# emdgroup/tnmf

Hardware: NVIDIA B200
Metric: sample-iterations/sec for 2-D shift-NMF MU at 1/2/4/8 B200; % of roofline (higher is better)
Workload: dtype f32

## Files before the change

### tnmf_b200/csrc/tc_gradw_ts.cu

```cuda
#include "tc_common.cuh"

namespace tnmf {
namespace tc {
namespace gwt {

using tiled::ceil_div;
using tiled::Geo2;
using tiled::round_up;

constexpr int kCT = 64;
constexpr int kNB = 16;
constexpr int kWorkers = 256;
#ifndef TNMF_GW_ISSUERS
#define TNMF_GW_ISSUERS 2
#endif
constexpr int kIssuers = TNMF_GW_ISSUERS;
constexpr int kThreads = 32 * (8 + kIssuers + 4);
constexpr int kEpoch = 8;
constexpr int kMaxAStages = 4;
constexpr int kRingMax = 24;
constexpr int kRawMax = 4;
constexpr int kMaxSmem = 226 * 1024;

struct Plan {
    int KPL;
    int TXP, RW, RWp, rawX, raw_floats, nraw;
    int KS, n_sub, n_astages, a_col0, NA;
    int RS, NRr, ring_floats;
    int tiles;
    long long total, quota, units;
    int round_robin;
    int grid;
    size_t smem;
};

struct Args {
    const float *V, *R, *H;
    float *partials;
    int m0;
};

bool make_plan(const Geo2 &g, Plan &p) {
    p = Plan();
    if (g.AY < 1 || g.AY > 14) return false;
    p.KPL = g.C * g.AX;
    if (p.KPL > 64) return false;
    p.NA = kNB * g.AY;
    const int spare = 512 - 2 * p.NA;
#ifdef TNMF_GW_KS16
    if (spare >= 2 * 32) p.KS = 16;
#else
    if (spare >= 2 * 64) p.KS = 32;
#endif
    else if (spare >= 2 * 32) p.KS = 16;
    else return false;
    p.n_sub = kCT / p.KS;
    p.n_astages = spare / (2 * p.KS);
    if (p.n_astages > kMaxAStages) p.n_astages = kMaxAStages;
    p.n_astages &= ~1;
    p.a_col0 = 2 * p.NA;
    p.TXP = g.TX + g.AX - 1;
    p.RW = kCT + g.AX - 1;
    p.RWp = p.RW + 1;
    while ((p.RWp - g.AX) % 32 != 0) ++p.RWp;
    p.rawX = round_up(g.C * p.RWp, 32);
    p.raw_floats = 2 * p.rawX + 128;
    p.nraw = ceil_div(2 * g.C * p.RW, kWorkers);
    if (p.nraw > kRawMax) return false;
    const size_t fixed = (size_t)2 * p.raw_floats * 4 + 1024;
    for (p.RS = kRingMax; p.RS >= g.AY + 1; --p.RS) {
        p.NRr = (p.RS + g.AY - 1) * kNB;
        p.ring_floats = (p.NRr * 4 + 4) * (kCT / 4);
        if (fixed + (size_t)2 * p.ring_floats * 4 <= (size_t)kMaxSmem) break;
    }
    if (p.RS < g.AY + 1) return false;
    p.smem = fixed + (size_t)2 * p.ring_floats * 4;
    const long long cols = (long long)g.N * p.TXP;
    if (cols <= 0 || cols >= (1ll << 31) - kCT) return false;
    p.tiles = (int)((cols + kCT - 1) / kCT);
    const int sms = tma::sm_count();
    p.total = (long long)p.tiles * g.TY;
    p.quota = (p.total + sms - 1) / sms;
    const long long min_quota = g.TY < 8 ? g.TY : 8;
    if (p.quota < min_quota) p.quota = min_quota;
    const long long whole = (p.tiles + sms - 1) / sms * (long long)g.TY;
    p.round_robin = (double)whole <= 1.1 * (double)(p.quota + 2 * (g.AY - 1));
    if (p.round_robin) {
        p.quota = g.TY;
        p.grid = p.tiles < sms ? p.tiles : sms;
        p.units = p.tiles;
        return true;
    }
    p.grid = (int)((p.total + p.quota - 1) / p.quota);
    p.units = (long long)p.grid * ((p.quota + g.TY - 2) / g.TY + 1);
    return true;
}

struct Unit {
    int tile, ty0, ty1, r_lo, r_hi;
};
__device__ __forceinline__ Unit make_unit(long long u, const Geo2 &g, const Plan &p) {
    Unit w;
    const long long b = u % p.grid, k = u / p.grid;
    const long long lo = p.round_robin ? u * (long long)g.TY : b * p.quota, hi = min(lo + p.quota, p.total);
    w.tile = p.round_robin ? (int)u : (int)(lo / g.TY + k);
    const long long t0 = (long long)w.tile * g.TY;
    const long long s0 = max(lo, t0), s1 = min(hi, t0 + g.TY);
    w.ty0 = s1 > s0 ? (int)(s0 - t0) : 0;
    w.ty1 = s1 > s0 ? (int)(s1 - t0) : 0;
    w.r_lo = max(0, w.ty0 - g.offy);
    w.r_hi = min(g.DY - 1, w.ty1 - 1 - g.offy + g.AY - 1);
    return w;
}

template <int KS>
__global__ void __launch_bounds__(kThreads, 1) gradw_ts_kernel(const Geo2 g, const Plan p, const Args a) {
    extern __shared__ __align__(128) float smem[];
    __shared__ __align__(8) unsigned long long a_full[kMaxAStages], a_empty[kMaxAStages], h_full[kRingMax], h_free[kRingMax],
        set_done[2], set_free[2];
    __shared__ unsigned tmem_base_s;
    constexpr int CPT = KS / 2;
    const int tid = threadIdx.x, warp = __shfl_sync(0xffffffffu, tid >> 5, 0), lane = tid & 31;
    const int AY = g.AY, AX = g.AX, C = g.C, RS = p.RS, RW = p.RW;
    float *ring_hi = smem, *ring_lo = smem + p.ring_floats;
    float *raw = ring_lo + p.ring_floats;

    if (tid == 0) {
        for (int s = 0; s < p.n_astages; ++s) { mbar_init(&a_full[s], 8); mbar_init(&a_empty[s], kIssuers); }
        for (int s = 0; s < kRingMax; ++s) { mbar_init(&h_full[s], kWorkers); mbar_init(&h_free[s], kIssuers); }
        for (int s = 0; s < 2; ++s) { mbar_init(&set_done[s], kIssuers); mbar_init(&set_free[s], 128); }
        mbar_fence_init();
    }
    if (warp == 8) tmem_alloc(&tmem_base_s, 512);
    for (int idx = tid; idx < 2 * p.raw_floats; idx += kThreads) raw[idx] = 0.f;
    tc_fence_before();
    __syncthreads();
    tc_fence_after();
    const unsigned tmem_base = tmem_base_s;
    if (warp < 4) {
        for (int c = 0; c < 512; c += 16) tmem_st16_zero(tmem_base + ((unsigned)(warp * 32) << 16) + (unsigned)c);
        tmem_st_wait();
    }
    tc_fence_before();
    __syncthreads();
    tc_fence_after();

    const long long count = (long long)g.M * C * AY * AX;

    if (warp < 8) {
        const int quarter = warp & 3, half = warp >> 2;
        const int L = quarter * 32 + lane;
        const int X = L >> 6, k = L & 63;
        const bool live = k < p.KPL;
        const bool warp_live = ((quarter * 32) & 63) < p.KPL;
        const int src_off = live ? X * p.rawX + (k / AX) * p.RWp + (k % AX) : 2 * p.rawX + 16;
        const unsigned t_lane = tmem_base + ((unsigned)(quarter * 32) << 16) + (unsigned)(p.a_col0 + half * CPT);
        int st = 0;
        unsigned ph = 0, buf = 0;
        TC_PROF_DECL(empty); TC_PROF_DECL(hfree); TC_PROF_DECL(bar); TC_PROF_DECL(total);
#ifdef TNMF_TC_PROFILE
        prof_total = -clock64();
#endif
        const long long plane = (long long)g.DY * g.DX;
        const int raw_count = 2 * C * RW;
        const int h_ml = tid >> 4, h_cg = tid & 15;
        int slot_new = 0;
        unsigned wraps = 0;
        for (long long u = blockIdx.x; u < p.units; u += gridDim.x) {
            const Unit w = make_unit(u, g, p);
            if (w.ty0 >= w.ty1) break;
            long long roff[kRawMax];
            int rdst[kRawMax];
#pragma unroll
            for (int e = 0; e < kRawMax; ++e) {
                roff[e] = -1;
                rdst[e] = -1;
                const int q = tid + kWorkers * e;
                if (e < p.nraw && q < raw_count) {
                    const int Xq = q / (C * RW), qq = q - Xq * (C * RW);
                    const int c = qq / RW, xr = qq - c * RW;
                    rdst[e] = Xq * p.rawX + c * p.RWp + xr;
                    const long long J = (long long)w.tile * kCT + xr;
                    const int n = (int)(J / p.TXP);
                    const int x = (int)(J - (long long)n * p.TXP) - g.offx;
                    if (n < g.N && (unsigned)x < (unsigned)g.DX) roff[e] = ((long long)n * C + c) * plane + x;
                }
            }
            long long hoff[4];
#pragma unroll
            for (int e = 0; e < 4; ++e) {
                const long long J = (long long)w.tile * kCT + 4 * h_cg + e;
                const int n = (int)(J / p.TXP);
                const int xv = (int)(J - (long long)n * p.TXP);
                hoff[e] = (n < g.N && xv < g.TX && a.m0 + h_ml < g.M)
                              ? (long long)n * g.hsn + (long long)(a.m0 + h_ml) * g.hsm + xv : -1;
            }
            float rv[kRawMax];
            auto load_raw = [&](int r) {
#pragma unroll
                for (int e = 0; e < kRawMax; ++e) {
                    const float *src = ((tid + kWorkers * e) >= C * RW) ? a.R : a.V;
                    rv[e] = roff[e] >= 0 ? __ldg(src + (long long)r * g.DX + roff[e]) : 0.f;
                }
            };
            auto load_h = [&](int ty) {
                float4 hv;
                hv.x = hoff[0] >= 0 ? a.H[hoff[0] + (long long)ty * g.hsy] : 0.f;
                hv.y = hoff[1] >= 0 ? a.H[hoff[1] + (long long)ty * g.hsy] : 0.f;
                hv.z = hoff[2] >= 0 ? a.H[hoff[2] + (long long)ty * g.hsy] : 0.f;
                hv.w = hoff[3] >= 0 ? a.H[hoff[3] + (long long)ty * g.hsy] : 0.f;
                return hv;
            };
            float4 hv_next = make_float4(0.f, 0.f, 0.f, 0.f);
            int hv_row = -1;
            int next_new = w.ty0;
            load_raw(w.r_lo);
            for (int r = w.r_lo; r <= w.r_hi; ++r) {
                const int t_b = min(w.ty1 - 1, r + g.offy);
                unsigned new_slots = 0;
                for (; next_new <= t_b; ++next_new) {
                    const int slot = slot_new;
                    const float4 hv = next_new == hv_row ? hv_next : load_h(next_new);
                    if (wraps) TC_PROF_WAIT(hfree, mbar_wait_backoff(&h_free[slot], (wraps - 1u) & 1u, 40));
                    if (++slot_new == RS) { slot_new = 0; ++wraps; }
                    float4 hi, lo;
                    split_tf32(hv.x, hi.x, lo.x); split_tf32(hv.y, hi.y, lo.y);
                    split_tf32(hv.z, hi.z, lo.z); split_tf32(hv.w, hi.w, lo.w);
                    const int nrow = slot * kNB + h_ml;
                    const size_t o = (size_t)(nrow >> 3) * 32 + (size_t)h_cg * (p.NRr * 4 + 4) + (size_t)(nrow & 7) * 4;
                    *reinterpret_cast<float4 *>(ring_hi + o) = hi;
                    *reinterpret_cast<float4 *>(ring_lo + o) = lo;
                    if (slot < AY - 1) {
                        const size_t om = o + (size_t)RS * (kNB / 8) * 32;
                        *reinterpret_cast<float4 *>(ring_hi + om) = hi;
                        *reinterpret_cast<float4 *>(ring_lo + om) = lo;
                    }
                    new_slots |= 1u << slot;
                }
                if (new_slots) {
                    fence_proxy_async();
                    for (; new_slots; new_slots &= new_slots - 1) mbar_arrive(&h_full[__ffs(new_slots) - 1]);
                }
                float *rb = raw + (size_t)buf * p.raw_floats;
#pragma unroll
                for (int e = 0; e < kRawMax; ++e)
                    if (rdst[e] >= 0) rb[rdst[e]] = rv[e];
                if (r < w.r_hi) load_raw(r + 1);
                if (next_new < w.ty1) { hv_next = load_h(next_new); hv_row = next_new; }
                TC_PROF_WAIT(bar, asm volatile("bar.sync 1, 256;\n" ::: "memory"));
                const float *src = rb + src_off + half * CPT;
                for (int h = 0; h < kCT / KS; ++h) {
                    TC_PROF_WAIT(empty, mbar_wait_backoff(&a_empty[st], ph ^ 1u, 20));
                    tc_fence_after();
                    if (warp_live) {
                        float hi[CPT], lo[CPT];
#pragma unroll
                        for (int j = 0; j < CPT; ++j) split_tf32(src[h * KS + j], hi[j], lo[j]);
                        const unsigned t = t_lane + (unsigned)(st * 2 * KS);
                        if constexpr (CPT == 16) {
                            tmem_st16(t, hi);
                            tmem_st16(t + KS, lo);
                        } else {
                            tmem_st8(t, hi);
                            tmem_st8(t + KS, lo);
                        }
                        tmem_st_wait();
                    }
                    tc_fence_before();
                    __syncwarp();
                    if (lane == 0) mbar_arrive(&a_full[st]);
                    if (++st == p.n_astages) { st = 0; ph ^= 1u; }
                }
                buf ^= 1u;
            }
        }
#ifdef TNMF_TC_PROFILE
        prof_total += clock64();
        if (blockIdx.x == 0 && tid == 0)
            printf("gradw_ts workers: total %lld  wait a_empty %lld  wait h_free %lld  raw barrier %lld\n", prof_total, prof_empty,
                   prof_hfree, prof_bar);
#endif
    } else if (warp >= 8 + kIssuers) {
        int rows_done = 0;
        bool first_drain = true;
        TC_PROF_DECL(done); TC_PROF_DECL(total);
#ifdef TNMF_TC_PROFILE
        prof_total = -clock64();
#endif
        auto drain = [&](int e) {
            const int set = (int)(e & 1);
            const int l = (warp & 3) * 32 + lane;
            const int X = l >> 6, k = l & 63;
            const bool live = k < p.KPL;
            const int c = live ? k / AX : 0, ax = live ? k - c * AX : 0;
            float *slice = a.partials + (long long)blockIdx.x * 2 * count + (long long)X * count;
            const unsigned tbase = tmem_base + ((unsigned)((warp & 3) * 32) << 16) + (unsigned)(set * p.NA);
            float old_next[kNB];
#pragma unroll
            for (int ml = 0; ml < kNB; ++ml) old_next[ml] = 0.f;
            if (live && !first_drain) {
                const float *nx = slice + (((long long)a.m0 * C + c) * AY + (AY - 1)) * AX + ax;
#pragma unroll
                for (int ml = 0; ml < kNB; ++ml) old_next[ml] = a.m0 + ml < g.M ? __ldcg(nx + ml * (long long)C * AY * AX) : 0.f;
            }
            TC_PROF_WAIT(done, mbar_wait_backoff(&set_done[set], (unsigned)((e >> 1) & 1), 100));
            tc_fence_after();
            const long long mstride = (long long)C * AY * AX;
            float *dst_base = slice + (((long long)a.m0 * C + c) * AY) * AX + ax;
            for (int j = 0; j < AY; ++j) {
                float v[16], old[kNB];
#pragma unroll
                for (int ml = 0; ml < kNB; ++ml) old[ml] = old_next[ml];
                if (j + 1 < AY && live && !first_drain) {
                    const float *nx = dst_base + (long long)(AY - 2 - j) * AX;
#pragma unroll
                    for (int ml = 0; ml < kNB; ++ml) old_next[ml] = a.m0 + ml < g.M ? __ldcg(nx + ml * mstride) : 0.f;
                }
                tmem_ld16(tbase + (unsigned)(j * kNB), v);
                tmem_ld_wait();
                tmem_st16_zero(tbase + (unsigned)(j * kNB));
                if (live) {
                    float *dst0 = dst_base + (long long)(AY - 1 - j) * AX;
#pragma unroll
                    for (int ml = 0; ml < kNB; ++ml)
                        if (a.m0 + ml < g.M) __stcg(dst0 + ml * mstride, v[ml] + old[ml]);
                }
            }
            tmem_st_wait();
            tc_fence_before();
            mbar_arrive(&set_free[set]);
            first_drain = false;
        };
        for (long long u = blockIdx.x; u < p.units; u += gridDim.x) {
            const Unit w = make_unit(u, g, p);
            if (w.ty0 >= w.ty1) break;
            rows_done += w.r_hi - w.r_lo + 1;
        }
        const int n_epochs = (rows_done + kEpoch - 1) / kEpoch;
        for (int e = 0; e < n_epochs; ++e) drain(e);
#ifdef TNMF_TC_PROFILE
        prof_total += clock64();
        if (blockIdx.x == 0 && tid == 32 * (8 + kIssuers))
            printf("gradw_ts drainers: total %lld  wait set_done %lld  (%d epochs)\n", prof_total, prof_done, n_epochs);
#endif
    } else {
        const unsigned tmem_u = __shfl_sync(0xffffffffu, tmem_base, 0);
        const unsigned lbo_b = (unsigned)p.NRr * 16 + 16;
        const unsigned desc_hi = (128u >> 4) | (1u << 14);
        const unsigned b_lo_word = ((lbo_b >> 4) << 16);
        const unsigned ring_hi16 = __shfl_sync(0xffffffffu, smem_u32(ring_hi) >> 4, 0);
        const unsigned ring_lo16 = __shfl_sync(0xffffffffu, smem_u32(ring_lo) >> 4, 0);
        const unsigned b_step16 = (2 * lbo_b) >> 4;
        const int X = warp - 8;
        const int j_lo = (AY * X + kIssuers - 1) / kIssuers, j_hi = (AY * (X + 1) + kIssuers - 1) / kIssuers - 1;
        int st = 0;
        unsigned ph = 0;
        int rows_done = 0;
        int slot_new = 0, slot_out = 0, slot_a = 0;
        unsigned par_new = 0;
        TC_PROF_DECL(full); TC_PROF_DECL(hfull); TC_PROF_DECL(setfree); TC_PROF_DECL(total); TC_PROF_DECL(issue); TC_PROF_DECL(commit); TC_PROF_DECL(commit2);
#ifdef TNMF_TC_PROFILE
        prof_total = -clock64();
#endif
        for (long long u = blockIdx.x; u < p.units; u += gridDim.x) {
            const Unit w = make_unit(u, g, p);
            if (w.ty0 >= w.ty1) break;
            int next_new = w.ty0, next_out = w.ty0, win0 = w.ty0;
            slot_a = slot_new;
            for (int r = w.r_lo; r <= w.r_hi; ++r) {
                const int epoch = rows_done / kEpoch;
                if (rows_done % kEpoch == 0 && epoch >= 2) {
                    TC_PROF_WAIT(setfree, mbar_wait(&set_free[epoch & 1], (unsigned)(((epoch >> 1) - 1) & 1)));
                    tc_fence_after();
                }
                const unsigned tset = tmem_u + (unsigned)((epoch & 1) * p.NA);
                const int ay_hi = min(AY - 1, r + g.offy - w.ty0);
                const int t_a = r + g.offy - ay_hi, t_b = min(w.ty1 - 1, r + g.offy);
                const int j0 = r + g.offy - AY + 1;
                for (; next_new <= t_b; ++next_new) {
                    TC_PROF_WAIT(hfull, mbar_wait(&h_full[slot_new], par_new));
                    if (++slot_new == RS) { slot_new = 0; par_new ^= 1u; }
                }
                for (; win0 < t_a; ++win0)
                    if (++slot_a == RS) slot_a = 0;
                const int ta_x = max(t_a, j0 + j_lo), tb_x = min(t_b, j0 + j_hi);
                const int cnt = tb_x - ta_x + 1;
                const unsigned col0 = tset + (unsigned)((ta_x - j0) * kNB);
                const unsigned idesc0 = idesc_tf32(128, kNB * max(cnt, 1));
                const unsigned b0 = (unsigned)(slot_a + (ta_x - t_a)) * 16u;
                for (int h = 0; h < kCT / KS; ++h) {
                    TC_PROF_WAIT(full, mbar_wait(&a_full[st], ph));
                    tc_fence_after();
#ifdef TNMF_TC_PROFILE
                    const long long t_i = clock64();
#endif
                    const unsigned ta_hi = tmem_u + (unsigned)(p.a_col0 + st * 2 * KS), ta_lo = ta_hi + KS;
                    if (cnt > 0 && elect_one()) {
#pragma unroll
                        for (int ks = 0; ks < KS / 8; ++ks) {
                            const unsigned kb = (unsigned)(h * (KS / 8) + ks) * b_step16 + b0;
                            const unsigned long long b_hi = ((unsigned long long)desc_hi << 32) | (b_lo_word | (ring_hi16 + kb));
                            const unsigned long long b_lo = ((unsigned long long)desc_hi << 32) | (b_lo_word | (ring_lo16 + kb));
                            mma_tf32_ts(col0, ta_hi + 8u * ks, b_hi, idesc0, 1u);
                            mma_tf32_ts(col0, ta_lo + 8u * ks, b_hi, idesc0, 1u);
                            mma_tf32_ts(col0, ta_hi + 8u * ks, b_lo, idesc0, 1u);
                        }
                    }
                    __syncwarp();
#ifdef TNMF_TC_PROFILE
                    prof_issue += clock64() - t_i;
#endif
                    TC_PROF_WAIT(commit, mma_commit_elect(&a_empty[st]));
                    if (++st == p.n_astages) { st = 0; ph ^= 1u; }
                }
                for (; next_out < w.ty1 && min(g.DY - 1, next_out - g.offy + AY - 1) <= r; ++next_out) {
                    TC_PROF_WAIT(commit2, mma_commit_elect(&h_free[slot_out]));
                    if (++slot_out == RS) slot_out = 0;
                }
                if (++rows_done % kEpoch == 0) mma_commit_elect(&set_done[epoch & 1]);
            }
        }
        if (rows_done % kEpoch != 0) mma_commit_elect(&set_done[(rows_done / kEpoch) & 1]);
#ifdef TNMF_TC_PROFILE
        prof_total += clock64();
        if (blockIdx.x == 0 && lane == 0)
            printf("gradw_ts mma %d: total %lld  wait a_full %lld  wait h_full %lld  wait set_free %lld  issuing %lld  commit a_empty %lld  commit h_free %lld (%d rows)\n",
                   X, prof_total, prof_full, prof_hfull, prof_setfree, prof_issue, prof_commit, prof_commit2, rows_done);
#endif
        __syncwarp();
    }
    tc_fence_before();
    __syncthreads();
    if (warp == 8) tmem_dealloc(tmem_base, 512);
}

template <int KS>
static int launch(const Geo2 &g, const Plan &p, const Args &a, cudaStream_t st) {
    auto kern = gradw_ts_kernel<KS>;
    cudaError_t e = cudaFuncSetAttribute(kern, cudaFuncAttributeMaxDynamicSharedMemorySize, kMaxSmem);
    if (e != cudaSuccess) return status_from_cuda(e);
    kern<<<(unsigned)p.grid, kThreads, p.smem, st>>>(g, p, a);
    TNMF_CHECK_LAUNCH();
    return TNMF_OK;
}

}
}

bool tc_gradw_ts_supported(const Geo &g, int dtype) {
    if (!tc::rank2_ok(g, dtype)) return false;
    tc::gwt::Plan p;
    return tc::gwt::make_plan(tiled::make_geo2(g), p);
}

size_t tc_gradw_ts_workspace_bytes(const Geo &g) {
    tc::gwt::Plan p;
    if (!tc::gwt::make_plan(tiled::make_geo2(g), p)) return 0;
    return (size_t)p.grid * 2 * (size_t)g.M * g.C * g.A[1] * g.A[2] * sizeof(float);
}

int tc_gradient_w_ts(const Geo &g, const float *V, const float *R, const float *H, float *neg, float *pos, void *workspace,
                     size_t workspace_bytes, cudaStream_t st) {
    const tiled::Geo2 q = tiled::make_geo2(g);
    tc::gwt::Plan p;
    if (!tc::gwt::make_plan(q, p)) return TNMF_EUNSUPPORTED;
    const long long count = (long long)g.M * g.C * g.A[1] * g.A[2];
    if (!workspace || workspace_bytes < tc_gradw_ts_workspace_bytes(g)) return TNMF_EWORKSPACE;
    tc::gwt::Args a;
    a.V = V; a.R = R; a.H = H; a.partials = (float *)workspace;
    for (int m0 = 0; m0 < g.M; m0 += tc::gwt::kNB) {
        a.m0 = m0;
        const int s = p.KS == 32 ? tc::gwt::launch<32>(q, p, a, st) : tc::gwt::launch<16>(q, p, a, st);
        if (s) return s;
    }
    return finish_gradient_w<float>((const float *)workspace, p.grid, count, neg, pos, st);
}

int tc_gradw_ts_launches(const Geo &g) { return tiled::ceil_div(g.M, tc::gwt::kNB) + 1; }

}
```

Before: 34740.

## Pack hi/lo TF32 splits into separate TMEM lanes when KPL fits 32

```diff
diff --git a/tnmf_b200/csrc/tc_gradw_ts.cu b/tnmf_b200/csrc/tc_gradw_ts.cu
--- a/tnmf_b200/csrc/tc_gradw_ts.cu
+++ b/tnmf_b200/csrc/tc_gradw_ts.cu
@@ -21,9 +21,14 @@
 constexpr int kRingMax = 24;
 constexpr int kRawMax = 4;
 constexpr int kMaxSmem = 226 * 1024;
+constexpr int kMaxLeft = 1;
+constexpr int kLeftRing = 16;
+constexpr int kXchg = 2 * 2 * kNB * 32;
+constexpr int kDrainers = 128;
 
 struct Plan {
     int KPL;
+    int hl, side;
     int TXP, RW, RWp, rawX, raw_floats, nraw;
     int KS, n_sub, n_astages, a_col0, NA;
     int RS, NRr, ring_floats;
@@ -40,24 +45,28 @@
     int m0;
 };
 
-bool make_plan(const Geo2 &g, Plan &p) {
+bool make_plan(const Geo2 &g, Plan &p, bool hl_ok = true) {
     p = Plan();
     if (g.AY < 1 || g.AY > 14) return false;
     p.KPL = g.C * g.AX;
     if (p.KPL > 64) return false;
+    p.hl = hl_ok && p.KPL <= 32 + kMaxLeft;
+    p.side = p.hl && p.KPL > 32;
     p.NA = kNB * g.AY;
     const int spare = 512 - 2 * p.NA;
+    if (p.hl) p.KS = 32;
 #ifdef TNMF_GW_KS16
-    if (spare >= 2 * 32) p.KS = 16;
+    else if (spare >= 2 * 32) p.KS = 16;
 #else
-    if (spare >= 2 * 64) p.KS = 32;
+    else if (spare >= 2 * 64) p.KS = 32;
 #endif
     else if (spare >= 2 * 32) p.KS = 16;
     else return false;
     p.n_sub = kCT / p.KS;
-    p.n_astages = spare / (2 * p.KS);
+    p.n_astages = spare / ((p.hl ? 1 : 2) * p.KS);
     if (p.n_astages > kMaxAStages) p.n_astages = kMaxAStages;
     p.n_astages &= ~1;
+    if (p.n_astages < 2) return false;
     p.a_col0 = 2 * p.NA;
     p.TXP = g.TX + g.AX - 1;
     p.RW = kCT + g.AX - 1;
@@ -67,13 +76,13 @@
     p.raw_floats = 2 * p.rawX + 128;
     p.nraw = ceil_div(2 * g.C * p.RW, kWorkers);
     if (p.nraw > kRawMax) return false;
-    const size_t fixed = (size_t)2 * p.raw_floats * 4 + 1024;
+    const size_t fixed = (size_t)2 * p.raw_floats * 4 + 1024 + (p.hl ? kXchg * 4 : 0) + (p.side ? kLeftRing * 128 * 4 : 0);
     for (p.RS = kRingMax; p.RS >= g.AY + 1; --p.RS) {
         p.NRr = (p.RS + g.AY - 1) * kNB;
         p.ring_floats = (p.NRr * 4 + 4) * (kCT / 4);
         if (fixed + (size_t)2 * p.ring_floats * 4 <= (size_t)kMaxSmem) break;
     }
-    if (p.RS < g.AY + 1) return false;
+    if (p.RS < g.AY + 1) return p.hl && make_plan(g, p, false);
     p.smem = fixed + (size_t)2 * p.ring_floats * 4;
     const long long cols = (long long)g.N * p.TXP;
     if (cols <= 0 || cols >= (1ll << 31) - kCT) return false;
@@ -113,22 +122,29 @@
     return w;
 }
 
-template <int KS>
+template <int KS, bool HL>
 __global__ void __launch_bounds__(kThreads, 1) gradw_ts_kernel(const Geo2 g, const Plan p, const Args a) {
     extern __shared__ __align__(128) float smem[];
     __shared__ __align__(8) unsigned long long a_full[kMaxAStages], a_empty[kMaxAStages], h_full[kRingMax], h_free[kRingMax],
-        set_done[2], set_free[2];
+        set_done[2], set_free[2], l_full[kLeftRing], l_empty[kLeftRing];
     __shared__ unsigned tmem_base_s;
     constexpr int CPT = KS / 2;
+    constexpr int kAYMax = 14;
+    static_assert(!HL || KS == 32, "the HL layout stages 32 columns");
     const int tid = threadIdx.x, warp = __shfl_sync(0xffffffffu, tid >> 5, 0), lane = tid & 31;
     const int AY = g.AY, AX = g.AX, C = g.C, RS = p.RS, RW = p.RW;
     float *ring_hi = smem, *ring_lo = smem + p.ring_floats;
     float *raw = ring_lo + p.ring_floats;
+    float *xchg = raw + 2 * p.raw_floats;
+    float *left = xchg + kXchg;
+    const bool side = HL && p.side;
+    const int left_off = (32 / AX) * p.RWp + 32 % AX;
 
     if (tid == 0) {
         for (int s = 0; s < p.n_astages; ++s) { mbar_init(&a_full[s], 8); mbar_init(&a_empty[s], kIssuers); }
-        for (int s = 0; s < kRingMax; ++s) { mbar_init(&h_full[s], kWorkers); mbar_init(&h_free[s], kIssuers); }
+        for (int s = 0; s < kRingMax; ++s) { mbar_init(&h_full[s], kWorkers); mbar_init(&h_free[s], kIssuers + (side ? kDrainers : 0)); }
         for (int s = 0; s < 2; ++s) { mbar_init(&set_done[s], kIssuers); mbar_init(&set_free[s], 128); }
+        for (int s = 0; s < kLeftRing; ++s) { mbar_init(&l_full[s], 128); mbar_init(&l_empty[s], kDrainers); }
         mbar_fence_init();
     }
     if (warp == 8) tmem_alloc(&tmem_base_s, 512);
@@ -150,14 +166,16 @@
     if (warp < 8) {
         const int quarter = warp & 3, half = warp >> 2;
         const int L = quarter * 32 + lane;
-        const int X = L >> 6, k = L & 63;
-        const bool live = k < p.KPL;
-        const bool warp_live = ((quarter * 32) & 63) < p.KPL;
-        const int src_off = live ? X * p.rawX + (k / AX) * p.RWp + (k % AX) : 2 * p.rawX + 16;
+        const int X = HL ? (quarter & 1) : L >> 6, k = HL ? lane : L & 63;
+        const bool part_lo = HL && quarter >= 2;
+        const bool live = k < (HL ? min(p.KPL, 32) : p.KPL);
+        const bool warp_live = HL || ((quarter * 32) & 63) < p.KPL;
+        const int src_off = live ? X * p.rawX + (k / AX) * p.RWp + (k % AX) : 2 * p.rawX + (HL ? 31 : 16);
         const unsigned t_lane = tmem_base + ((unsigned)(quarter * 32) << 16) + (unsigned)(p.a_col0 + half * CPT);
         int st = 0;
         unsigned ph = 0, buf = 0;
-        TC_PROF_DECL(empty); TC_PROF_DECL(hfree); TC_PROF_DECL(bar); TC_PROF_DECL(total);
+        unsigned lrow = 0;
+        TC_PROF_DECL(empty); TC_PROF_DECL(hfree); TC_PROF_DECL(bar); TC_PROF_DECL(lempty); TC_PROF_DECL(total);
 #ifdef TNMF_TC_PROFILE
         prof_total = -clock64();
 #endif
@@ -252,7 +270,18 @@
                 for (int h = 0; h < kCT / KS; ++h) {
                     TC_PROF_WAIT(empty, mbar_wait_backoff(&a_empty[st], ph ^ 1u, 20));
                     tc_fence_after();
-                    if (warp_live) {
+                    if constexpr (HL) {
+                        float v[CPT], d;
+                        if (part_lo) {
+#pragma unroll
+                            for (int j = 0; j < CPT; ++j) split_tf32(src[h * KS + j], d, v[j]);
+                        } else {
+#pragma unroll
+                            for (int j = 0; j < CPT; ++j) split_tf32(src[h * KS + j], v[j], d);
+                        }
+                        tmem_st16(t_lane + (unsigned)(st * KS), v);
+                        tmem_st_wait();
+                    } else if (warp_live) {
                         float hi[CPT], lo[CPT];
 #pragma unroll
                         for (int j = 0; j < CPT; ++j) split_tf32(src[h * KS + j], hi[j], lo[j]);
@@ -271,27 +300,37 @@
                     if (lane == 0) mbar_arrive(&a_full[st]);
                     if (++st == p.n_astages) { st = 0; ph ^= 1u; }
                 }
+                if (side && tid < 128) {
+                    const unsigned ls = lrow % kLeftRing;
+                    if (lrow >= kLeftRing) TC_PROF_WAIT(lempty, mbar_wait_backoff(&l_empty[ls], (lrow / kLeftRing - 1u) & 1u, 20));
+                    left[ls * 128 + tid] = rb[(tid >> 6) * p.rawX + left_off + (tid & 63)];
+                    mbar_arrive(&l_full[ls]);
+                }
+                ++lrow;
                 buf ^= 1u;
             }
         }
 #ifdef TNMF_TC_PROFILE
         prof_total += clock64();
         if (blockIdx.x == 0 && tid == 0)
-            printf("gradw_ts workers: total %lld  wait a_empty %lld  wait h_free %lld  raw barrier %lld\n", prof_total, prof_empty,
-                   prof_hfree, prof_bar);
+            printf("gradw_ts workers: total %lld  wait a_empty %lld  wait h_free %lld  raw barrier %lld  wait l_empty %lld\n",
+                   prof_total, prof_empty, prof_hfree, prof_bar, prof_lempty);
 #endif
     } else if (warp >= 8 + kIssuers) {
+        const int di = tid - 32 * (8 + kIssuers);
         int rows_done = 0;
         bool first_drain = true;
-        TC_PROF_DECL(done); TC_PROF_DECL(total);
+        unsigned xpar = 0;
+        TC_PROF_DECL(done); TC_PROF_DECL(lfull); TC_PROF_DECL(hfull); TC_PROF_DECL(side); TC_PROF_DECL(total);
 #ifdef TNMF_TC_PROFILE
         prof_total = -clock64();
 #endif
         auto drain = [&](int e) {
             const int set = (int)(e & 1);
             const int l = (warp & 3) * 32 + lane;
-            const int X = l >> 6, k = l & 63;
-            const bool live = k < p.KPL;
+            const int X = HL ? (l >> 5) & 1 : l >> 6, k = HL ? lane : l & 63;
+            const bool owner = !HL || l < 64;
+            const bool live = owner && k < (HL ? min(p.KPL, 32) : p.KPL);
             const int c = live ? k / AX : 0, ax = live ? k - c * AX : 0;
             float *slice = a.partials + (long long)blockIdx.x * 2 * count + (long long)X * count;
             const unsigned tbase = tmem_base + ((unsigned)((warp & 3) * 32) << 16) + (unsigned)(set * p.NA);
@@ -319,6 +358,19 @@
                 tmem_ld16(tbase + (unsigned)(j * kNB), v);
                 tmem_ld_wait();
                 tmem_st16_zero(tbase + (unsigned)(j * kNB));
+                if constexpr (HL) {
+                    float *xb = xchg + (xpar & 1u) * (kXchg / 2) + X * (kXchg / 4) + lane;
+                    xpar ^= 1u;
+                    if (!owner) {
+#pragma unroll
+                        for (int ml = 0; ml < kNB; ++ml) xb[ml * 32] = v[ml];
+                    }
+                    asm volatile("bar.sync 2, 128;\n" ::: "memory");
+                    if (owner) {
+#pragma unroll
+                        for (int ml = 0; ml < kNB; ++ml) v[ml] += xb[ml * 32];
+                    }
+                }
                 if (live) {
                     float *dst0 = dst_base + (long long)(AY - 1 - j) * AX;
 #pragma unroll
@@ -331,17 +383,91 @@
             mbar_arrive(&set_free[set]);
             first_drain = false;
         };
+        const int sx = di >> 6, sm = (di >> 2) & 15, sq = di & 3;
+        int slot_out = 0;
+        unsigned par_out = 0, lrow = 0;
+        bool first_unit = true;
         for (long long u = blockIdx.x; u < p.units; u += gridDim.x) {
             const Unit w = make_unit(u, g, p);
             if (w.ty0 >= w.ty1) break;
-            rows_done += w.r_hi - w.r_lo + 1;
+            float acc[kAYMax];
+#pragma unroll
+            for (int ay = 0; ay < kAYMax; ++ay) acc[ay] = 0.f;
+            int next_out = w.ty0;
+            const unsigned lrow0 = lrow;
+            unsigned lfree = lrow;
+            for (int r = w.r_lo; r <= w.r_hi; ++r, ++lrow) {
+                if (side) {
+#ifdef TNMF_TC_PROFILE
+                    const long long t_s = clock64();
+#endif
+                    TC_PROF_WAIT(lfull, mbar_wait_backoff(&l_full[lrow % kLeftRing], (lrow / kLeftRing) & 1u, 20));
+                    for (; next_out < w.ty1 && min(g.DY - 1, next_out - g.offy + AY - 1) <= r; ++next_out) {
+                        const int t = next_out;
+                        TC_PROF_WAIT(hfull, mbar_wait_backoff(&h_full[slot_out], par_out, 20));
+                        float hv[16];
+                        {
+                            const int nrow = slot_out * kNB + sm;
+                            const size_t o = (size_t)(nrow >> 3) * 32 + (size_t)sq * (p.NRr * 4 + 4) + (size_t)(nrow & 7) * 4;
+#pragma unroll
+                            for (int i = 0; i < 4; ++i) {
+                                const size_t oi = o + (size_t)(4 * i) * (p.NRr * 4 + 4);
+                                const float4 h = *reinterpret_cast<const float4 *>(ring_hi + oi);
+                                const float4 l = *reinterpret_cast<const float4 *>(ring_lo + oi);
+                                hv[4 * i] = h.x + l.x; hv[4 * i + 1] = h.y + l.y; hv[4 * i + 2] = h.z + l.z; hv[4 * i + 3] = h.w + l.w;
+                            }
+                        }
+                        mbar_arrive(&h_free[slot_out]);
+                        if (++slot_out == RS) { slot_out = 0; par_out ^= 1u; }
+                        const int ay_lo = max(0, g.offy - t), ay_hi = min(AY - 1, g.DY - 1 - t + g.offy);
+                        const unsigned l0row = lrow0 + (unsigned)(t - g.offy - w.r_lo);
+#pragma unroll
+                        for (int ay = 0; ay < kAYMax; ++ay) {
+                            if (ay < ay_lo || ay > ay_hi) continue;
+                            const float *lr = left + ((l0row + (unsigned)ay) % kLeftRing) * 128 + sx * 64 + 4 * sq;
+                            float s = acc[ay];
+#pragma unroll
+                            for (int i = 0; i < 4; ++i) {
+                                const float4 x = *reinterpret_cast<const float4 *>(lr + 16 * i);
+                                s = fmaf(hv[4 * i], x.x, s); s = fmaf(hv[4 * i + 1], x.y, s);
+                                s = fmaf(hv[4 * i + 2], x.z, s); s = fmaf(hv[4 * i + 3], x.w, s);
+                            }
+                            acc[ay] = s;
+                        }
+                    }
+                    for (; (int)(lfree - lrow0) <= r - (AY - 1) - w.r_lo; ++lfree) mbar_arrive(&l_empty[lfree % kLeftRing]);
+#ifdef TNMF_TC_PROFILE
+                    prof_side += clock64() - t_s;
+#endif
+                }
+                if (++rows_done % kEpoch == 0) drain(rows_done / kEpoch - 1);
+            }
+            if (side) {
+                for (; lfree != lrow; ++lfree) mbar_arrive(&l_empty[lfree % kLeftRing]);
+                unsigned cta;
+                asm volatile("mov.u32 %0, %%ctaid.x;\n" : "=r"(cta));
+                const int cL = 32 / AX, axL = 32 % AX;
+                float *dst = a.partials + (long long)cta * 2 * count + (long long)sx * count +
+                             (((long long)(a.m0 + sm) * C + cL) * AY) * AX + axL;
+#pragma unroll
+                for (int ay = 0; ay < kAYMax; ++ay) {
+                    float s = acc[ay];
+                    s += __shfl_xor_sync(0xffffffffu, s, 2);
+                    s += __shfl_xor_sync(0xffffffffu, s, 1);
+                    if (ay < AY && sq == 0 && a.m0 + sm < g.M) {
+                        float *d = dst + (long long)ay * AX;
+                        __stcg(d, first_unit ? s : __ldcg(d) + s);
+                    }
+                }
+            }
+            first_unit = false;
         }
-        const int n_epochs = (rows_done + kEpoch - 1) / kEpoch;
-        for (int e = 0; e < n_epochs; ++e) drain(e);
+        if (rows_done % kEpoch != 0) drain(rows_done / kEpoch);
 #ifdef TNMF_TC_PROFILE
         prof_total += clock64();
-        if (blockIdx.x == 0 && tid == 32 * (8 + kIssuers))
-            printf("gradw_ts drainers: total %lld  wait set_done %lld  (%d epochs)\n", prof_total, prof_done, n_epochs);
+        if (blockIdx.x == 0 && di == 0)
+            printf("gradw_ts drainers: total %lld  wait set_done %lld  leftover taps %lld (wait l_full %lld  wait h_full %lld)  (%d rows)\n",
+                   prof_total, prof_done, prof_side, prof_lfull, prof_hfull, rows_done);
 #endif
     } else {
         const unsigned tmem_u = __shfl_sync(0xffffffffu, tmem_base, 0);
@@ -394,16 +520,21 @@
 #ifdef TNMF_TC_PROFILE
                     const long long t_i = clock64();
 #endif
-                    const unsigned ta_hi = tmem_u + (unsigned)(p.a_col0 + st * 2 * KS), ta_lo = ta_hi + KS;
+                    const unsigned ta_hi = tmem_u + (unsigned)(p.a_col0 + st * (HL ? 1 : 2) * KS), ta_lo = ta_hi + KS;
                     if (cnt > 0 && elect_one()) {
 #pragma unroll
                         for (int ks = 0; ks < KS / 8; ++ks) {
                             const unsigned kb = (unsigned)(h * (KS / 8) + ks) * b_step16 + b0;
                             const unsigned long long b_hi = ((unsigned long long)desc_hi << 32) | (b_lo_word | (ring_hi16 + kb));
                             const unsigned long long b_lo = ((unsigned long long)desc_hi << 32) | (b_lo_word | (ring_lo16 + kb));
-                            mma_tf32_ts(col0, ta_hi + 8u * ks, b_hi, idesc0, 1u);
-                            mma_tf32_ts(col0, ta_lo + 8u * ks, b_hi, idesc0, 1u);
-                            mma_tf32_ts(col0, ta_hi + 8u * ks, b_lo, idesc0, 1u);
+                            if constexpr (HL) {
+                                mma_tf32_ts(col0, ta_hi + 8u * ks, b_hi, idesc0, 1u);
+                                mma_tf32_ts(col0, ta_hi + 8u * ks, b_lo, idesc0, 1u);
+                            } else {
+                                mma_tf32_ts(col0, ta_hi + 8u * ks, b_hi, idesc0, 1u);
+                                mma_tf32_ts(col0, ta_lo + 8u * ks, b_hi, idesc0, 1u);
+                                mma_tf32_ts(col0, ta_hi + 8u * ks, b_lo, idesc0, 1u);
+                            }
                         }
                     }
                     __syncwarp();
@@ -434,9 +565,9 @@
     if (warp == 8) tmem_dealloc(tmem_base, 512);
 }
 
-template <int KS>
+template <int KS, bool HL>
 static int launch(const Geo2 &g, const Plan &p, const Args &a, cudaStream_t st) {
-    auto kern = gradw_ts_kernel<KS>;
+    auto kern = gradw_ts_kernel<KS, HL>;
     cudaError_t e = cudaFuncSetAttribute(kern, cudaFuncAttributeMaxDynamicSharedMemorySize, kMaxSmem);
     if (e != cudaSuccess) return status_from_cuda(e);
     kern<<<(unsigned)p.grid, kThreads, p.smem, st>>>(g, p, a);
@@ -470,7 +601,8 @@
     a.V = V; a.R = R; a.H = H; a.partials = (float *)workspace;
     for (int m0 = 0; m0 < g.M; m0 += tc::gwt::kNB) {
         a.m0 = m0;
-        const int s = p.KS == 32 ? tc::gwt::launch<32>(q, p, a, st) : tc::gwt::launch<16>(q, p, a, st);
+        const int s = p.hl ? tc::gwt::launch<32, true>(q, p, a, st)
+                      : p.KS == 32 ? tc::gwt::launch<32, false>(q, p, a, st) : tc::gwt::launch<16, false>(q, p, a, st);
         if (s) return s;
     }
     return finish_gradient_w<float>((const float *)workspace, p.grid, count, neg, pos, st);
```

Result: slower. 22690 (median of 6 runs) (-34.7%).
